# harvardinformatics/IMCoalHMM

Measured on AMD Instinct MI355X. Metric: alignment columns/sec (forward pass), 20-state isolation HMM, higher is better.
Workload: dtype f64

## Files before the change

### imcoalhmm_amd/csrc/imcoal_fwd.hip

```cpp
#include <hip/hip_runtime.h>

#include <algorithm>
#include <cerrno>
#include <climits>
#include <cmath>
#include <cstdint>
#include <cstdio>
#include <cstdlib>
#include <cstring>
#include <list>
#include <atomic>
#include <chrono>
#include <map>
#include <set>
#include <memory>
#include <mutex>
#include <condition_variable>
#include <string>
#include <vector>

#include <unistd.h>

#include "../../include/imcoal_fwd.h"
#include "kernels_plain.hpp"
// ... 59 lines not shown
    uint16_t *d_left = nullptr, *d_right = nullptr;
    uint16_t *d_order = nullptr;
    std::vector<uint16_t> order;
    std::vector<int> depth;
    uint64_t trained_on = 0;
    pid_t pid = 0;
    ~DictDev()
    {
        if (pid == getpid()) { dev_free(d_left); dev_free(d_right); dev_free(d_order); }
    }
};

struct Ev3 { hipEvent_t a, b, c; };

struct Ctx {
    pid_t pid = 0;
    int device = -1;
    bool ready = false;
    hipStream_t stream = nullptr;
    int cus = 256;
    uint64_t next_obs_id = 1, next_dict_id = 1;
    size_t seg_override = 0;
    int compression = 1;
    int kernel_pref = 0;
    bool profile = false;
    bool rank1_handoff = true;
    int blocked_variant = 4;
    int wide_blocked = -1;
    int z4_stream = -1;
    bool table_pairs = true;
    int table_triples = -1;
    bool table_split = true;
    int table_split_max = -1;
    bool xcd_affine = true;
    int fuse_tail = 1;
    bool fuse_head = true;
    bool pack_table = true;
    bool guard = false;
    bool use_graphs = false;
    std::vector<Ev3> events;
    std::map<int, std::shared_ptr<DictDev>> dicts;
    uint64_t last_plan[8] = {0, 0, 0, 0, 0, 0, 0, 0};
    uint64_t r1_checked = 0, r1_collapsed = 0;
    std::string last_kernels;
} g;

void drop_plans();
void reset_kernel_attributes();
void model_release();

int ensure_ctx()
{
    const pid_t me = getpid();
    if (g.ready && g.pid == me) return IMC_OK;
    if (g.ready && g.pid != me)
        return fail(IMC_ERR_HIP, "libimcoal_fwd was initialised in the parent process before fork(): fork the chain "
                                 "processes before the first imc_* call of the parent, or use the spawn start method");
    int n = 0;
    if (hipGetDeviceCount(&n) != hipSuccess || n <= 0)
        return fail(IMC_ERR_NODEVICE, "no HIP device available (libimcoal_fwd has no CPU fallback)");
    if (g.device < 0) {
        int cur = 0;
        if (hipGetDevice(&cur) != hipSuccess) cur = 0;
        g.device = cur;
    }
    if (g.device >= n) return fail(IMC_ERR_NODEVICE, "requested device index out of range");
    HIP_TRY(hipSetDevice(g.device));
    hipDeviceProp_t prop;
    HIP_TRY(hipGetDeviceProperties(&prop, g.device));
    if (std::strncmp(prop.gcnArchName, "gfx950", 6) != 0)
        return fail(IMC_ERR_NODEVICE, std::string("device is ") + prop.gcnArchName + ", this library is built for gfx950 only");
    g.cus = prop.multiProcessorCount > 0 ? prop.multiProcessorCount : 256;
    HIP_TRY(hipStreamCreateWithFlags(&g.stream, hipStreamNonBlocking));
    g.use_graphs = std::getenv("IMC_GRAPH") != nullptr;
    if (const char *gd = std::getenv("IMC_GUARD")) g.guard = std::atoi(gd) != 0;
    if (const char *bv = std::getenv("IMC_BLOCKED")) { const int v = std::atoi(bv); if (v >= 2 && v <= 5) g.blocked_variant = v; }
    if (const char *r1 = std::getenv("IMC_RANK1")) g.rank1_handoff = std::atoi(r1) != 0;
    if (const char *pt = std::getenv("IMC_PACK_TABLE")) g.pack_table = std::atoi(pt) != 0;
    if (const char *tp = std::getenv("IMC_TABLE_PAIRS")) g.table_pairs = std::atoi(tp) != 0;
    if (const char *fh = std::getenv("IMC_FUSE_HEAD")) g.fuse_head = std::atoi(fh) != 0;
    if (const char *ts = std::getenv("IMC_TABLE_SPLIT")) g.table_split = std::atoi(ts) != 0;
    if (const char *tm = std::getenv("IMC_TABLE_SPLIT_MAX")) g.table_split_max = std::max(0, std::atoi(tm));
    if (const char *tt = std::getenv("IMC_TABLE_TRIPLES")) g.table_triples = std::atoi(tt) != 0 ? 1 : 0;
    if (const char *ft = std::getenv("IMC_FUSE_TAIL")) g.fuse_tail = std::max(0, std::min(2, std::atoi(ft)));
    if (const char *xa = std::getenv("IMC_XCD_AFFINE")) g.xcd_affine = std::atoi(xa) != 0;
    if (const char *wb = std::getenv("IMC_WIDE_BLOCKED")) { const int v = std::atoi(wb); if (v >= -1 && v <= 1) g.wide_blocked = v; }
    if (const char *zs = std::getenv("IMC_Z4_STREAM")) { const int v = std::atoi(zs); if (v >= -1 && v <= 1) g.z4_stream = v; }
    g.pid = me;
    g.ready = true;
    return IMC_OK;
}

struct GuardRec { hipDeviceptr_t va; size_t va_size; hipMemGenericAllocationHandle_t handle; hipDeviceptr_t map; size_t map_size; };
std::map<void *, GuardRec> &g_guard = *new std::map<void *, GuardRec>();

hipError_t dev_alloc(void **p, size_t bytes)
{
    bytes = std::max<size_t>(bytes, 16);
    if (!g.guard) return hipMalloc(p, bytes);
    hipMemAllocationProp prop{};
    prop.type = hipMemAllocationTypePinned;
    prop.location.type = hipMemLocationTypeDevice;
    prop.location.id = g.device;
    size_t gran = 0;
    hipError_t e = hipMemGetAllocationGranularity(&gran, &prop, hipMemAllocationGranularityMinimum);
    if (e != hipSuccess || gran == 0) return e != hipSuccess ? e : hipErrorUnknown;
    GuardRec r{};
    r.map_size = (bytes + gran - 1) / gran * gran;
    r.va_size = r.map_size + 2 * gran;
    e = hipMemAddressReserve(&r.va, r.va_size, gran, nullptr, 0);
    if (e != hipSuccess) return e;
    e = hipMemCreate(&r.handle, r.map_size, &prop, 0);
    if (e != hipSuccess) { (void)hipMemAddressFree(r.va, r.va_size); return e; }
    r.map = (hipDeviceptr_t)((char *)r.va + gran);
    e = hipMemMap(r.map, r.map_size, 0, r.handle, 0);
    if (e == hipSuccess) {
        hipMemAccessDesc ad{};
        ad.location = prop.location;
// ... 10 lines not shown

void dev_free(void *p)
{
    if (!p) return;
    auto it = g_guard.find(p);
    if (it == g_guard.end()) { (void)hipFree(p); return; }
    (void)hipDeviceSynchronize();
    (void)hipMemUnmap(it->second.map, it->second.map_size);
    (void)hipMemRelease(it->second.handle);
    g_guard.erase(it);
}

}

struct imc_obs {
    uint64_t id;
    pid_t pid;
    int device;
    int nsym;
    size_t L;
    uint8_t *d_sym;
    bool wide_raw;
    std::shared_ptr<DictDev> dict;
    uint8_t *d_tok[imc::kNumLevels];
    bool wide[imc::kNumLevels];
    size_t ntok[imc::kNumLevels];
    int alphabet[imc::kNumLevels];
    std::vector<uint32_t> tok_count[imc::kNumLevels];
};

namespace {

constexpr size_t OBS_PAD = 256;

hipError_t upload_padded(const uint8_t *host, size_t n, uint8_t **dptr)
{
    const size_t bytes = ((n + OBS_PAD - 1) / OBS_PAD) * OBS_PAD + OBS_PAD;
    hipError_t e = dev_alloc((void **)dptr, bytes);
    if (e != hipSuccess) return e;
    e = hipMemsetAsync(*dptr, 0, bytes, g.stream);
    if (e == hipSuccess && n) e = hipMemcpyAsync(*dptr, host, n, hipMemcpyHostToDevice, g.stream);
    if (e == hipSuccess) e = hipStreamSynchronize(g.stream);
    return e;
}

void release_tokens(imc_obs *o)
{
    for (int l = 0; l < imc::kNumLevels; ++l) {
        bool alias = false;
        for (int m = 0; m < l; ++m) alias |= (o->d_tok[m] == o->d_tok[l]);
        if (o->d_tok[l] && !alias) dev_free(o->d_tok[l]);
    }
    for (int l = 0; l < imc::kNumLevels; ++l) {
        o->d_tok[l] = nullptr; o->wide[l] = false; o->ntok[l] = 0; o->alphabet[l] = o->nsym; o->tok_count[l].clear();
    }
    o->dict.reset();
}

void obs_release(imc_obs *o)
{
    dev_free(o->d_sym);
    release_tokens(o);
}

size_t wide_min_count(size_t sample_tokens)
{
// ... 141 lines not shown
    return IMC_OK;
}


using ChainFn = void (*)(const ChainDesc *, int, const uint32_t *, uint32_t, uint32_t, const double *, const int *,
                         const int *, uint32_t, double *, int *, double *, int);

struct KernelChoice {
    int R, G, NP, VPW, minw;
    void (*plain)(PropArgs);
    void (*zip)(PropArgs);
    size_t (*zip_lds)(int);
    ChainFn chain;
    bool zip_attr_set;
    void (*big_table_raw)(BigArgs);
    void (*big_table_level)(BigArgs, const uint16_t *, int);
    void (*big_prop)(BigArgs, const BigBlock *);
    int big_prop_waves;
    void (*big_vec)(BigArgs, const BigBlock *, int, int);
    void (*big_vec_tail)(BigArgs, const BigBlock *, int, int);
    int big_vec_waves;
    int big_nslab;
    size_t big_lds;
    void (*zip2)(BigArgs);
    size_t (*zip2_lds)(int);
    bool zip2_attr_set;
    bool plain_attr_set = false;
    void (*zip3)(BigArgs) = nullptr;
    size_t (*zip3_lds)(int) = nullptr;
    bool zip3_attr_set = false;
    void (*zip4)(BigArgs) = nullptr;
    void (*zip4w)(BigArgs) = nullptr;
    void (*zip4s)(BigArgs) = nullptr, (*zip4sw)(BigArgs) = nullptr;
    void (*zip4_raw)(BigArgs) = nullptr;
    void (*zip4_level)(BigArgs, int, int) = nullptr;
    void (*zip4_level2)(BigArgs, const int4 *, int, int, const double *) = nullptr;
    void (*zip4_level2_first)(BigArgs, const int4 *, int, int, const double *) = nullptr;
    void (*zip4_level2_split)(BigArgs, const int4 *, int, int, const double *) = nullptr;
    void (*zip4_level2_split_first)(BigArgs, const int4 *, int, int, const double *) = nullptr;
    void (*zip4_level3)(BigArgs, const int4 *, int, int, const double *) = nullptr;
    void (*zip4_level3_first)(BigArgs, const int4 *, int, int, const double *) = nullptr;
    size_t (*zip4_level3_lds)(size_t) = nullptr;
    size_t (*zip4_lds)(int, int) = nullptr;
    int (*zip4_max_hot)(int, size_t) = nullptr;
    int tok_doubles = 0;
    int z4_waves = Z2WAVES;
    bool wide_blocked = false;
    int z4_slots() const { return z4_waves * 4; }
    bool chain_self_emax = false;
    bool zip4_attr_set = false, zip4w_attr_set = false, zip4s_attr_set = false, zip4sw_attr_set = false, zip4_attr_l3 = false;
    bool use3() const;
    size_t blocked_lds(int A) const { return use3() ? zip3_lds(A) : zip2_lds(A); }
};

template <int R, int G, int MW>
KernelChoice make_kc()
{
    constexpr int NP = R * G;
    KernelChoice k{R, G, NP, 64 / G, MW, k_propagate<R, G, MW>, k_zpropagate<R, G>, &ZipGeom<R, G>::lds_bytes,
                   k_chain<NP, (NP <= 12 ? 6 : NP <= 24 ? 4 : NP <= 32 ? 3 : NP <= 64 ? 2 : 1)>, false, nullptr, nullptr, nullptr, 0, nullptr, nullptr, 0, 0, 0, nullptr, nullptr, false};
    k.chain_self_emax = true;
    if constexpr (NP % 4 == 0 && NP <= 24) {
        k.zip2 = k_zpropagate2<NP / 4>;
        k.zip2_lds = &Zip2Geom<NP / 4>::lds_bytes;
        k.zip3 = k_zpropagate3<NP / 4>;
        k.zip3_lds = &Zip3Geom<NP / 4>::lds_bytes;
        k.tok_doubles = Zip3Geom<NP / 4>::TOK;
        if constexpr (NP <= 24) {
            k.zip4 = k_zpropagate4<NP / 4, false, true>;
            k.zip4w = k_zpropagate4<NP / 4, true, true>;
            k.zip4s = k_zpropagate4<NP / 4, false, false>;
            k.zip4sw = k_zpropagate4<NP / 4, true, false>;
            k.zip4_raw = k_z4_raw<NP / 4>;
            k.zip4_level = k_z4_level<NP / 4>;
            k.zip4_level2 = k_z4_level2<NP / 4, false>;
            k.zip4_level2_first = k_z4_level2<NP / 4, true>;
            k.zip4_level2_split = k_z4_level2<NP / 4, false, Z4_SPLIT_WAVES>;
            k.zip4_level2_split_first = k_z4_level2<NP / 4, true, Z4_SPLIT_WAVES_FIRST>;
            k.zip4_level3 = k_z4_level3<NP / 4, false>;
            k.zip4_level3_first = k_z4_level3<NP / 4, true>;
            k.zip4_level3_lds = &Z4L3Geom<NP / 4>::lds_bytes;
            k.zip4_lds = &Zip4Geom<NP / 4>::lds_bytes;
            k.zip4_max_hot = &Zip4Geom<NP / 4>::max_hot;
        }
    }
    if constexpr (NP == 28 || NP == 32) {
        k.tok_doubles = Zip3Geom<NP / 4>::TOK;
        k.zip4s = k_zpropagate4<NP / 4, false, false>;
        k.zip4sw = k_zpropagate4<NP / 4, true, false>;
        k.zip4_raw = k_z4_raw<NP / 4>;
        k.zip4_level = k_z4_level<NP / 4>;
        k.zip4_lds = &Zip4Geom<NP / 4>::lds_bytes;
        k.z4_waves = Zip4Shape<NP / 4>::WAVES;
        k.wide_blocked = true;
    }
    return k;
}

template <int NT, int NSLAB>
KernelChoice make_big()
{
    constexpr int NP = 16 * NT;
    constexpr bool dealt = NT > 4 && NT % 4 != 0;
    void (*prop)(BigArgs, const BigBlock *) = k_big_propagate<NT, NSLAB>;
    if constexpr (dealt) prop = k_big_propagate_s<NT, NSLAB>;
    return KernelChoice{0, NT, NP, 0, 1, nullptr, nullptr, nullptr, k_chain<NP, 0>, false, k_big_table_raw<NT>,
                        k_big_table_level<NT>, prop, dealt ? BS_WAVES : NT, k_big_vector<NT, false>, k_big_vector<NT, true>, BigVec<NT>::WAVES, NSLAB,
                        BigSlab<NT, NSLAB>::bytes, nullptr, nullptr, false};
}

bool KernelChoice::use3() const { return zip3 && g.blocked_variant >= 3; }

KernelChoice kChoices[] = {
    make_kc<4, 1, 2>(), make_kc<4, 2, 2>(), make_kc<4, 3, 2>(), make_kc<4, 4, 2>(), make_kc<4, 5, 2>(),
    make_kc<3, 8, 2>(), make_kc<2, 14, 2>(), make_kc<2, 16, 2>(), make_kc<2, 20, 1>(), make_kc<1, 48, 1>(),
    make_kc<1, 56, 1>(), make_kc<1, 64, 1>(),
    make_big<6, 1>(), make_big<7, 1>(), make_big<8, 2>(), make_big<9, 3>(), make_big<10, 2>(), make_big<12, 3>(), make_big<14, 7>(),
    make_big<16, 8>(),
};
constexpr int IMC_MAX_N = 256;

KernelChoice kMidChoices[] = {make_big<2, 1>(), make_big<3, 1>(), make_big<4, 1>()};

KernelChoice *choose_kernel(int N, bool prefer_gemm)
{
    if (prefer_gemm && N > 24 && N <= 64)
        for (auto &k : kMidChoices)
            if (k.NP >= N) return &k;
    for (auto &k : kChoices)
        if (k.NP >= N) return &k;
    return nullptr;
}

void reset_kernel_attributes()
{
    for (auto &k : kChoices) k.zip4_attr_l3 = k.zip_attr_set = k.zip2_attr_set = k.zip3_attr_set = k.zip4_attr_set = k.zip4w_attr_set = k.zip4s_attr_set = k.zip4sw_attr_set = k.plain_attr_set = false;
    for (auto &k : kMidChoices) k.zip4_attr_l3 = k.zip_attr_set = k.zip2_attr_set = k.zip3_attr_set = k.zip4_attr_set = k.zip4w_attr_set = k.zip4s_attr_set = k.zip4sw_attr_set = k.plain_attr_set = false;
}


struct Group {
    bool big = false;
    bool bigvec = false;
    bool zip2 = false;
    std::vector<uint32_t> seg_ids, seg_out;
    std::vector<Z2Block> blocks;
    std::vector<BigBlock> big_blocks;
    BigBlock *d_big_blocks = nullptr;
    uint32_t *d_seg_ids = nullptr, *d_seg_out = nullptr;
    Z2Block *d_blocks = nullptr;
    bool zip4 = false;
    bool wide_tokens = false;
    bool stream_table = false;
    int n_hot = 0;
    std::vector<uint16_t> hot;
    uint16_t *d_hot = nullptr;
    uint16_t *d_tab_order = nullptr;
    int *d_tab_lvl = nullptr;
    int4 *d_tab_desc = nullptr;
    int4 *d_tab_desc2 = nullptr;
    std::vector<std::pair<int, int>> tab2;
    std::vector<Z2Tail> tails;
    Z2Tail *d_tails = nullptr;
    double *d_tailX = nullptr;
    int *d_tailE = nullptr, *d_tail_arrive = nullptr;
    int tail_stride = 0;
    int4 *d_tab_desc3 = nullptr;
    std::vector<std::pair<int, int>> tab3;
    std::vector<int> tab_lvl;
// ... 367 lines not shown
                size_t lmax = 0;
                for (size_t L : lens) lmax = std::max(lmax, L);
                const double np2 = (double)kc->NP * kc->NP, per_cu_steps = (double)total * B / (double)g.cus;
                const double cost_vec = std::max((double)lmax * (np2 / 4.5 + 1500.0), per_cu_steps * matvec_step_cycles(np2, gr.A));
                double cost_gemm = std::max(16.0, per_cu_steps) * gemm_cu_step_cycles(kc->NP);
                if (g.rank1_handoff && !g.seg_override && gr.seglen >= R1_MIN_SEGLEN) {
                    const HandoffEstimate he = estimate_handoff((double)gr.seglen, std::max(1.0, (double)total / gr.seglen), B,
                                                                (double)handoff_head(gr), kc->NP, kc->big_nslab, gr.A, g.cus);
                    if (he.m) cost_gemm = std::min(cost_gemm, he.cycles);
                }
                if (std::getenv("IMC_DEBUG"))
                    std::fprintf(stderr, "[imc] plan: GEMM chain seg %zu cost %.3g cycles; mat-vec chain cost %.3g cycles\n",
                                 gr.seglen, cost_gemm, cost_vec);
                if (!op_mode && (g.kernel_pref == 1 || (g.kernel_pref == 0 && (cost_vec < cost_gemm || lmax <= gr.seglen)))) {
                    gr.bigvec = true;
                    gr.seglen = std::max<size_t>(16, round_up(lmax, 16));
                }
                if (gr.zip) gr.model_us = gr.model_tab_us + (gr.bigvec ? cost_vec : cost_gemm) / 2200.0;
            } else {
                double cost_vec = 0.0;
                size_t seg_vec;
                if (gr.zip) {
                    const double lds_cycles = ((double)kc->R * kc->NP / 2 + kc->NP / 2.0) * 4.0 + kc->R * 6.0 + 40.0;
                    seg_vec = choose_seglen(lens, N, B, kc->VPW, (double)g.cus * ZWAVES, lds_cycles * ZWAVES, &cost_vec);
                } else {
                    seg_vec = choose_seglen(lens, N, B, kc->VPW, (double)g.cus * 4.0 * kc->minw,
                                            kc->minw * 1.7 * (4.0 * kc->R * kc->NP + 16.0), &cost_vec);
                }
                gr.seglen = seg_vec;
                if ((kc->zip2 || (wide && gr.zip4)) && g.kernel_pref != 1 && (gr.zip4 || kc->blocked_lds(gr.A) <= LDS_BUDGET) && (gr.zip || (S == gr.A && S <= imc::kByteAlphabet))) {
                    const int SL = kc->z4_slots(), WV = kc->z4_waves;
                    size_t total = 0;
                    for (size_t L : lens) total += L;
                    const bool two_per_cu = gr.zip4 && kc->use3() && kc->NP <= 12 &&
                                            z4_streamed((double)B * (gr.A + 1) * kc->tok_doubles * 8.0, B);
                    const double rows = (double)g.cus * SL * (two_per_cu ? 2.0 : 1.0);
                    const double rb = kc->NP / 4.0;
                    const double step_cycles = (mfma() ? 25.5 * rb * rb * rb * 0.55 : 5.8 * rb * rb * kc->NP) * (two_per_cu ? 1.85 : 1.0);
                    size_t seg_blk = 16;
                    double slots = 0.0, cost_blk = 1e300;
                    const bool can_pack = mfma() && !op_mode;
                    auto rows_used = [&](size_t sg) {
                        double r = 0.0, singles = 0.0;
                        for (size_t L : lens) {
                            if (!L) continue;
                            const double nseg = std::ceil((double)L / (double)sg);
                            if (nseg <= 1.0 && can_pack) singles += 1.0;
                            else r += std::ceil(nseg / SL) * SL;
                        }
                        return r + std::ceil(singles / SL) * SL;
                    };
                    size_t lmax = 0;
                    for (size_t L : lens) lmax = std::max(lmax, L);
                    std::vector<size_t> cands;
                    for (int rounds = 1; rounds <= 16; ++rounds) {
                        const double target = std::max((double)SL, std::floor(rows * rounds / B));
                        size_t sg = std::max<size_t>(16, round_up((size_t)std::ceil((double)total / target), Z2GRAN));
                        int it = 0;
                        for (; it < 1024 && rows_used(sg) > target && sg < lmax + 16; ++it) sg += Z2GRAN;
                        if (rows_used(sg) > target) continue;
                        cands.push_back(sg);
                    }
                    for (size_t u = 1; u <= 8; ++u)
                        cands.push_back(std::max<size_t>(16, round_up((lmax + SL * u - 1) / (SL * u), Z2GRAN)));
                    {
                        std::vector<size_t> sorted(lens);
                        std::sort(sorted.begin(), sorted.end());
                        const size_t med = sorted[sorted.size() / 2];
                        for (size_t u = 1; u <= 4; ++u)
                            cands.push_back(std::max<size_t>(16, round_up((med + SL * u - 1) / (SL * u), Z2GRAN)));
                        for (size_t fixed_len : {16, 32, 48, 64, 96, 128, 192}) cands.push_back(fixed_len);
                        if (can_pack)
                            for (size_t qi : {sorted.size() / 2, sorted.size() * 9 / 10, sorted.size() - 1})
                                cands.push_back(std::max<size_t>(16, round_up(sorted[qi], Z2GRAN)));
                    }
                    for (size_t sg : cands) {
                        const double table = !mfma() ? (double)(gr.A - S) * (400.0 + (double)kc->NP * kc->NP * kc->NP / 64.0)
                                             : gr.zip4 ? 9000.0 : 2600.0 * std::min(12.0, (double)(gr.A - S));
                        const double fixed = table + 5.0 * (WV / 4.0) * step_cycles;
                        for (size_t cand : {sg, round_up(sg, 16)}) {
                            const double u = rows_used(cand);
                            double c = std::ceil(u * B / rows) * ((double)cand * (WV / 4.0) * step_cycles + fixed + (cand % 16 ? 7700.0 : 0.0));
                            if (can_pack && cand >= lmax) c *= 1.15;
                            if (c < cost_blk) { cost_blk = c; seg_blk = cand; slots = u; }
                        }
                    }
                    if (std::getenv("IMC_DEBUG"))
                        std::fprintf(stderr, "[imc] plan: vector kernel seg %zu cost %.3g cycles; blocked kernel seg %zu slots %.0f cost %.3g cycles\n",
                                     seg_vec, cost_vec, seg_blk, slots, cost_blk);
                    const bool vec_fits = !gr.zip || kc->zip_lds(gr.A) <= LDS_BUDGET;
                    if (g.kernel_pref == 2 || cost_blk < cost_vec || !vec_fits || gr.zip4) { gr.zip2 = true; gr.seglen = seg_blk; }
                }
                if (gr.zip && !gr.zip2) gr.model_us = gr.model_tab_us + cost_vec / 2200.0;
            }
            if (g.seg_override) gr.seglen = round_up(std::max<size_t>(g.seg_override, 16), 16);
            if (gr.bigvec)
                for (size_t L : lens) gr.bigvec = gr.bigvec && L <= gr.seglen && !op_mode;
            if (gr.big && !gr.bigvec && g.rank1_handoff && gr.seglen >= R1_MIN_SEGLEN) {
                double cols = 0.0, toks = 0.0;
                for (int f : gr.chunks) { cols += (double)chunks[f]->L; toks += (double)(gr.zip ? chunks[f]->ntok[gr.level] : chunks[f]->L); }
                const double span = toks > 0.0 ? cols / toks : 1.0;
                const size_t head = handoff_head(gr);
                const double nseg = std::max(1.0, toks / (double)gr.seglen);
                if (g.seg_override) {
                    if (gr.seglen >= 4 * R1_MIN_HEAD) {
                        gr.rank1 = true;
                        gr.head_len = (int)round_up(gr.seglen / 4, 16);
                        gr.checkpoints.assign(1, gr.head_len);
                    }
                } else {
                    const int best_m = estimate_handoff((double)gr.seglen, nseg, B, (double)head, kc->NP, kc->big_nslab, gr.A, g.cus).m;
                    if (best_m) {
                        gr.rank1 = true;
                        gr.head_len = (int)head;
                        gr.seglen = std::max<size_t>(16, round_up(gr.seglen / best_m, 16));
                        size_t c = round_up(std::max<size_t>(64, (size_t)(R1_HEAD_MIN_COLUMNS / span)), 16);
                        while ((int)gr.checkpoints.size() < R1_MAX_ROUNDS && c + gr.seglen / 8 < gr.seglen) {
                            gr.checkpoints.push_back((int)c);
                            const size_t step = (double)c * span < R1_DENSE_COLUMNS ? c / 8 : c / 2;
                            c = round_up(c + std::max<size_t>(16, step), 16);
                        }
                        if (gr.checkpoints.empty()) gr.rank1 = false;
                    }
                }
            }
        }
    }

    void cut_segments()
    {
        chunk_seg.assign(n_chunks + 1, 0);
        for (int f = 0; f < n_chunks; ++f) {
            chunk_seg[f] = (uint32_t)segs.size();
            const Group &gr = p->groups[chunk_group[f]];
            const size_t L = gr.zip ? chunks[f]->ntok[gr.level] : chunks[f]->L;
            const uint8_t *base = gr.zip ? chunks[f]->d_tok[gr.level] : chunks[f]->d_sym;
            if (!L) continue;
            const size_t K0 = (L + gr.seglen - 1) / gr.seglen;
            const size_t sl = round_up((L + K0 - 1) / K0, gr.zip2 ? Z2GRAN : 16);
            for (size_t off = 0, k = 0; off < L; off += sl, ++k) {
                const bool wide = gr.zip ? chunks[f]->wide[gr.level] : chunks[f]->wide_raw;
                const bool fst = k == 0 && !op_mode;
                segs.push_back(SegDesc{base + off * (wide ? 2 : 1), (uint32_t)std::min(sl, L - off),
                                       (fst ? SEG_FIRST : 0u) | (wide ? SEG_WIDE : 0u)});
                seg_first.push_back(fst);
            }
        }
        chunk_seg[n_chunks] = (uint32_t)segs.size();
    }

    int make_units()
    {
        chunk_units.assign(n_chunks, {});
        for (int f = 0; f < n_chunks; ++f) {
            const Group &gr = p->groups[chunk_group[f]];
            const uint32_t step = gr.zip2 ? (uint32_t)kc->z4_slots() : 1u;
            for (uint32_t sid = chunk_seg[f]; sid < chunk_seg[f + 1]; sid += step)
                chunk_units[f].push_back({sid, std::min(step, chunk_seg[f + 1] - sid)});
        }
        chunk_unit.assign(n_chunks + 1, 0);
        for (int f = 0; f < n_chunks; ++f) chunk_unit[f + 1] = chunk_unit[f] + (uint32_t)chunk_units[f].size();
        unit_vec0.assign(chunk_unit[n_chunks], 0);
        unit_first.assign(chunk_unit[n_chunks], 0);
        for (Group &gr : p->groups) {
            gr.vec_begin = (uint32_t)vecs.size();
            for (int f : gr.chunks) {
                gr.stream_len += gr.zip ? chunks[f]->ntok[gr.level] : chunks[f]->L;
                for (size_t u = 0; u < chunk_units[f].size(); ++u) {
                    const uint32_t sid = chunk_units[f][u].first, ns = chunk_units[f][u].second;
                    const uint32_t uid = chunk_unit[f] + (uint32_t)u;
                    const bool fst = seg_first[sid] != 0;
                    unit_first[uid] = fst;
// ... 593 lines not shown
                        head = false;
                        HIP_TRY(hipGetLastError());
                    }
                } else if (g.table_pairs && gr.d_tab_desc2 && kc->zip4_level2) {
                    bool head = fuse_head;
                    const size_t split_max = g.table_split_max >= 0 ? (size_t)g.table_split_max : (size_t)4 * g.cus;
                    for (const auto &lc : gr.tab2) {
                        if (g.table_split && (size_t)lc.second * B <= split_max) {
                            if (head)
                                hipLaunchKernelGGL(kc->zip4_level2_split_first, dim3((unsigned)(lc.second + Z4_SPLIT_WAVES_FIRST - 1) / Z4_SPLIT_WAVES_FIRST, (unsigned)B),
                                                   dim3(Z4_SPLIT_WAVES_FIRST * 64), p->pstride * 8, stream, ba,
                                                   (const int4 *)gr.d_tab_desc2, lc.first, lc.second, (const double *)p->h_params_dev[p->slot]);
                            else
                                hipLaunchKernelGGL(kc->zip4_level2_split, dim3((unsigned)(lc.second + Z4_SPLIT_WAVES - 1) / Z4_SPLIT_WAVES, (unsigned)B),
                                                   dim3(Z4_SPLIT_WAVES * 64), 0, stream, ba,
                                                   (const int4 *)gr.d_tab_desc2, lc.first, lc.second, (const double *)nullptr);
                            split_used = true;
                        } else if (head)
                            hipLaunchKernelGGL(kc->zip4_level2_first, dim3((unsigned)(lc.second + 3) / 4, (unsigned)B), dim3(64),
                                               p->pstride * 8, stream, ba,
                                               (const int4 *)gr.d_tab_desc2, lc.first, lc.second, (const double *)p->h_params_dev[p->slot]);
                        else
                            hipLaunchKernelGGL(kc->zip4_level2, dim3((unsigned)(lc.second + 3) / 4, (unsigned)B), dim3(64), 0, stream, ba,
                                               (const int4 *)gr.d_tab_desc2, lc.first, lc.second, (const double *)nullptr);
                        head = false;
                        HIP_TRY(hipGetLastError());
                    }
                } else
                for (int d = 0; d < gr.tab_nlvl; ++d) {
                    const int first = gr.tab_lvl[d], count = gr.tab_lvl[d + 1] - first;
                    hipLaunchKernelGGL(kc->zip4_level, dim3((unsigned)(count + 3) / 4, (unsigned)B), dim3(64), 0, stream, ba, first, count);
                    HIP_TRY(hipGetLastError());
                }
                void (*scan)(BigArgs) = gr.stream_table ? (gr.wide_tokens ? kc->zip4sw : kc->zip4s) : (gr.wide_tokens ? kc->zip4w : kc->zip4);
                bool &attr4 = gr.stream_table ? (gr.wide_tokens ? kc->zip4sw_attr_set : kc->zip4s_attr_set)
                                              : (gr.wide_tokens ? kc->zip4w_attr_set : kc->zip4_attr_set);
                if (!attr4) {
                    HIP_TRY(hipFuncSetAttribute((const void *)scan, hipFuncAttributeMaxDynamicSharedMemorySize, (int)LDS_BUDGET));
                    attr4 = true;
                }
                IMC_MARK_A();
                dim3 scan_grid(ba.n_group_segs, (unsigned)B);
                if (g.xcd_affine && B > 1) {
                    int first = 0, wg = 0;
                    auto phase = [&](int sets, int n_sets_total) {
                        ba.ph_begin[ba.n_phases] = wg; ba.ph_first[ba.n_phases] = first; ba.ph_sets[ba.n_phases] = sets;
                        ++ba.n_phases;
                        const int nb = (int)ba.n_group_segs;
                        wg += sets >= 8 ? 8 * nb * (n_sets_total / 8) : 8 * ((nb + 8 / sets - 1) / (8 / sets));
                        first += n_sets_total;
                    };
                    if (B >= 8) phase(8, B / 8 * 8);
                    for (int sets : {4, 2, 1})
                        if ((B % 8) & sets) phase(sets, sets);
                    scan_grid = dim3((unsigned)wg);
                }
                hipLaunchKernelGGL(scan, scan_grid, dim3(kc->z4_waves * 64), kc->zip4_lds(gr.A, gr.n_hot), stream, ba);
                note(std::string("k_zpropagate4<") + std::to_string(NP / 4) + (gr.wide_tokens ? ",16" : "") + (gr.stream_table ? ",streamed>" : ">") + strm);
                lp[4] = gr.seglen; lp[5] += gr.vsteps * (uint64_t)B; lp[6] += gr.stream_len; lp[7] = std::max(lp[7], (uint64_t)gr.A);
                HIP_TRY(hipGetLastError());
                continue;
            }
            const bool v3 = kc->use3();
            bool &attr_set = v3 ? kc->zip3_attr_set : kc->zip2_attr_set;
            if (!attr_set) {
                HIP_TRY(hipFuncSetAttribute((const void *)(v3 ? kc->zip3 : kc->zip2), hipFuncAttributeMaxDynamicSharedMemorySize,
                                            (int)LDS_BUDGET));
                attr_set = true;
            }
            size_t lds3 = kc->blocked_lds(gr.A);
            if (direct_params) { ba.params_src = p->h_params_dev[p->slot]; lds3 = ((lds3 + 15) & ~(size_t)15) + p->pstride * 8; }
            hipLaunchKernelGGL(v3 ? kc->zip3 : kc->zip2, dim3(ba.n_group_segs, (unsigned)B), dim3(Z2WAVES * 64), lds3, stream, ba);
            note(std::string(v3 ? "k_zpropagate3<" : "k_zpropagate2<") + std::to_string(NP / 4) + ">" + strm);
            if (gr.zip) { lp[4] = gr.seglen; lp[5] += gr.vsteps * (uint64_t)B; lp[6] += gr.stream_len; lp[7] = std::max(lp[7], (uint64_t)gr.A); }
            else { lp[2] = gr.seglen; lp[3] += gr.vsteps * (uint64_t)B; }
        } else if (gr.zip) {
            const size_t lds = kc->zip_lds(gr.A);
            if (!kc->zip_attr_set) {
                HIP_TRY(hipFuncSetAttribute((const void *)kc->zip, hipFuncAttributeMaxDynamicSharedMemorySize,
                                            (int)LDS_BUDGET));
                kc->zip_attr_set = true;
            }
            const uint32_t vpb = (uint32_t)(ZWAVES * kc->VPW);
            dim3 grid((gr.n_vecs + vpb - 1) / vpb, (unsigned)B);
            hipLaunchKernelGGL(kc->zip, grid, dim3(ZWAVES * 64), lds, stream, a);
            note("k_zpropagate<" + std::to_string(kc->R) + "," + std::to_string(kc->G) + ">" + strm);
            lp[4] = gr.seglen; lp[5] += gr.vsteps * (uint64_t)B; lp[6] += gr.stream_len; lp[7] = std::max(lp[7], (uint64_t)gr.A);
        } else {
            const uint32_t vpb = (uint32_t)(WPB * kc->VPW);
            dim3 grid((gr.n_vecs + vpb - 1) / vpb, (unsigned)B);
            const size_t lds = ((size_t)WPB * kc->VPW * NP + (size_t)S * NP) * 8;
// ... 1036 lines not shown
```

### imcoalhmm_amd/csrc/kernels_zip4.hpp

```cpp
#pragma once
#include "kernels_zip3.hpp"

template <int NT>
struct Zip4Shape {
    static constexpr int WAVES = NT <= 6 ? Z2WAVES : 4;
    static constexpr int SLOTS = WAVES * 4;
    static constexpr bool SLOT_MAP = NT <= 6;
};

template <int NT>
struct Zip4Geom {
    using G3 = Zip3Geom<NT>;
    static constexpr int TOK = G3::TOK;
    static constexpr int SLOTS = Zip4Shape<NT>::SLOTS;
    static constexpr int MAPS = Zip4Shape<NT>::SLOT_MAP ? 2 : 1;
    static constexpr int slots(int H) { return (H + 1 > SLOTS + 1 ? H + 1 : SLOTS + 1); }
    static constexpr size_t lds_bytes(int A, int H) { return (size_t)slots(H) * TOK * 8 + (size_t)(MAPS * (A + 2) + 64) * 4 + 16; }
    static constexpr int max_hot(int A, size_t budget)
    {
        const size_t fixed = (size_t)(MAPS * (A + 2) + 64) * 4 + 16;
        const size_t n = budget > fixed ? (budget - fixed) / ((size_t)TOK * 8) : 0;
        return n > 1 ? (int)n - 1 : 0;
    }
};

template <int NT>
__device__ __forceinline__ void zip4_step_regs(const double (&Pin)[NT][NT], double (&Pout)[NT][NT], const double (&Areg)[NT][NT])
{
#pragma unroll
    for (int I = 0; I < NT; ++I)
#pragma unroll
        for (int K = 0; K < NT; ++K)
#pragma unroll
            for (int J = 0; J < NT; ++J)
                Pout[I][J] = __builtin_amdgcn_mfma_f64_4x4x4f64(Areg[I][K], Pin[K][J], K == 0 ? 0.0 : Pout[I][J], 0, 0, 0);
}

template <int NT>
__device__ __forceinline__ void zip4_load_row_global(double (&a)[NT], const double *Gz, int I, int lo, int lx)
{
// ... 458 lines not shown
    const double *Cz = C + (size_t)max(cur.s, 0) * TOK, *Cn = C + (size_t)max(nxt.s, 0) * TOK;
#pragma unroll
    for (int I = 0; I < NT; ++I) {
        double an[NT], av[NT];
        if constexpr (HYB) {
            if (I + 1 < NT) zip3_load_row<NT>(an, Cz, I + 1, lo, lx);
            else zip3_load_row<NT>(an, Cn, 0, lo, lx);
        }
#pragma unroll
        for (int K = 0; K < NT; ++K) av[K] = cur_cold ? pre[I % ROWS][K] : al[K];
        __builtin_amdgcn_sched_barrier(0);
#pragma unroll
        for (int K = 0; K < NT; ++K)
#pragma unroll
            for (int J = 0; J < NT; ++J)
                Pout[I][J] = __builtin_amdgcn_mfma_f64_4x4x4f64(av[K], Pin[K][J], K == 0 ? 0.0 : Pout[I][J], 0, 0, 0);
        __builtin_amdgcn_sched_barrier(0);
        if (I + ROWS < NT) zip4_load_row_global<NT>(pre[I % ROWS], Gt + (size_t)cur.tok * TOK, I + ROWS, lo, lx);
        else zip4_load_row_global<NT>(pre[I % ROWS], Gn, I + ROWS - NT, lo, lx);
        if constexpr (HYB) {
#pragma unroll
            for (int K = 0; K < NT; ++K) al[K] = an[K];
        }
    }
}

#ifdef IMC_Z4_TIMING
__device__ long long g_z4_dbg[1024 * 8 * 3];
#define Z4_STAMP(k_) do { if (threadIdx.x == 0 && blockIdx.x < 1024 && blockIdx.y == 0) g_z4_dbg[blockIdx.x * 8 + (k_)] = wall_clock64(); } while (0)
#else
#define Z4_STAMP(k_) do { } while (0)
#endif

template <int NT, bool WIDE, bool HYB>
__global__ __launch_bounds__(Zip4Shape<NT>::WAVES * 64, Zip4Shape<NT>::WAVES / 4) void k_zpropagate4(BigArgs a)
{
    constexpr int TB = WIDE ? 2 : 1;
    using Geo = Zip3Geom<NT>;
    using G4 = Zip4Geom<NT>;
    constexpr int SLOTS = Zip4Shape<NT>::SLOTS;
    constexpr bool SLOT_MAP = Zip4Shape<NT>::SLOT_MAP;
    static_assert(SLOT_MAP || !HYB, "the hybrid form needs the slot map");
    constexpr int NP = Geo::NP, TOK = Geo::TOK, THREADS = Zip4Shape<NT>::WAVES * 64;
    extern __shared__ __attribute__((aligned(16))) double lds[];
    const int H = HYB ? a.n_hot : 0;
    double *C = lds;
    int *cex = reinterpret_cast<int *>(C + (size_t)G4::slots(H) * TOK);
    int *slot_of = cex + a.A + 2;
    int *xex = SLOT_MAP ? slot_of + a.A + 2 : slot_of;

    const int tid = threadIdx.x;
    int b = (int)blockIdx.y, bx = (int)blockIdx.x;
    if (a.n_phases > 0) {
        int ph = 0;
        while (ph + 1 < a.n_phases && (int)blockIdx.x >= a.ph_begin[ph + 1]) ++ph;
        const int local = (int)blockIdx.x - a.ph_begin[ph], xcd = local & 7, turn = local >> 3, nb = (int)a.n_group_segs;
        const int sets = a.ph_sets[ph];
        if (sets >= 8) {
            b = a.ph_first[ph] + xcd + 8 * (turn / nb);
            bx = turn % nb;
        } else {
            b = a.ph_first[ph] + xcd % sets;
            bx = turn * (8 / sets) + xcd / sets;
            if (bx >= nb) return;
        }
    }
    const double *pp = a.params + (size_t)b * a.pstride;
    const double *pi_p = pp;
    const double *Etg = pp + a.PP + (size_t)a.PP * a.PP;
    const double *Gt = a.Ctab + (size_t)b * (a.A + 1) * TOK;
    const int *Gc = a.cex + (size_t)b * (a.A + 1);
    const int IDENT = a.A;
    const double *Gi = Gt + (size_t)IDENT * TOK;

    Z4_STAMP(0);
    for (int z = tid; z <= a.A; z += THREADS) { cex[z] = Gc[z]; if constexpr (SLOT_MAP) slot_of[z] = -1; }
    if constexpr (HYB) {
        __syncthreads();
        for (int k = tid; k <= H; k += THREADS) slot_of[k < H ? (int)a.hot[k] : IDENT] = k;
        for (int idx = tid; idx < (H + 1) * (TOK / 2); idx += THREADS) {
            const int k = idx / (TOK / 2), w = idx - k * (TOK / 2);
            const int z = k < H ? (int)a.hot[k] : IDENT;
            reinterpret_cast<double2 *>(C + (size_t)k * TOK)[w] = reinterpret_cast<const double2 *>(Gt + (size_t)z * TOK)[w];
        }
    }
    __syncthreads();

    Z4_STAMP(1);
    const int lane = tid & 63;
    const int q = lane >> 4, bq = (lane >> 2) & 3, r = lane & 3;
    const int lo = (q * 4 + r) * Geo::NTE, lx = q * 4 + r;
    const Z2Block blk = a.blocks[bx];
    const int slot = (tid >> 6) * 4 + bq;
    const bool valid = slot < (int)blk.n;
    const uint32_t seg = blk.seg0 + (valid ? slot : ((slot & ~3) < (int)blk.n ? (slot & ~3) : 0));
    const SegDesc sd = a.segs[seg];
    const int len = valid ? (int)sd.len : 0;
    const bool first = (sd.first & SEG_FIRST) != 0;
    const uint8_t *tokp = sd.obs;
    typedef const __attribute__((address_space(1))) uint8_t *gptr;
    typedef uint32_t u32x4 __attribute__((ext_vector_type(4)));
    typedef const __attribute__((address_space(1))) u32x4 *gptr4;
    typedef const __attribute__((address_space(1))) uint32_t *gptr1;
    const gptr tokg = (gptr)tokp;

    double P[NT][NT], Q[NT][NT];
    {
        const int tok0 = (valid && first) ? seg_token(tokp, WIDE, 0) : 0;
#pragma unroll
        for (int K = 0; K < NT; ++K)
#pragma unroll
            for (int J = 0; J < NT; ++J) {
                const int i = 4 * K + q, c = 4 * J + r;
                double v;
                if (first) v = (c == 0 && i < a.N) ? pi_p[i] * Etg[(size_t)tok0 * a.PP + i] : 0.0;
                else v = (i == c && i < a.N) ? 1.0 : 0.0;
                P[K][J] = valid ? v : 0.0;
            }
    }
    int ex = 0;
    const int maxlen = wave_max_i32(len);
// ... 36 lines not shown
        }
        ex += t0.ce + t1.ce;
    };
    constexpr int PER = WIDE ? 8 : 16;
    auto masked_run = [&](int bi, int u0, int n) __attribute__((always_inline)) {
        uint4 ob = make_uint4(0u, 0u, 0u, 0u);
        if (bi * RESCALE_EVERY + u0 < len) {
            const u32x4 v = *(gptr4)(tokg + ((size_t)bi * RESCALE_EVERY + u0) * TB);
            ob = make_uint4(v.x, v.y, v.z, v.w);
        }
        const int live = len - bi * RESCALE_EVERY - u0;
        const int dead0 = (first && bi == 0 && u0 == 0) ? 0 : -1;
        const unsigned long long lo64 = (unsigned long long)ob.y << 32 | ob.x, hi64 = (unsigned long long)ob.w << 32 | ob.z;
        auto tok_of = [&](int v) __attribute__((always_inline)) {
            const unsigned long long h = v < PER / 2 ? lo64 : hi64;
            const int tk = WIDE ? (int)((h >> (16 * (v & 3))) & 0xffffull) : (int)((h >> (8 * (v & 7))) & 0xffull);
            return (v < live && v != dead0 && v < PER) ? tk : IDENT;
        };
        Z4Tok c0 = mk(tok_of(0)), c1 = mk(tok_of(1));
        prime(c0, c1);
#pragma unroll 1
        for (int v = 0; v < n; v += 2) {
            const Z4Tok c2 = mk(tok_of(v + 2)), c3 = mk(tok_of(v + 3));
            two_steps(c0, c1, c2, c3);
            c0 = c2;
            c1 = c3;
        }
    };
    auto masked_block = [&](int bi, int npos) __attribute__((always_inline)) {
#pragma unroll 1
        for (int u0 = 0; u0 < npos; u0 += PER) masked_run(bi, u0, min(PER, npos - u0));
        zip3_rescale<NT>(P, ex);
    };
    if (nfull == 0 && maxlen > 0) masked_block(0, min(RESCALE_EVERY, (maxlen + 1) & ~1));
    Z4_STAMP(2);
    if (nfull > 0) {
        constexpr int NW = 4 * TB;
        constexpr uint32_t TM = WIDE ? 0xffffu : 0xffu;
        auto load_words = [&](int bi, uint32_t (&w)[NW]) __attribute__((always_inline)) {
            gptr4 src = (gptr4)(tokg + (size_t)bi * RESCALE_EVERY * TB);
            const u32x4 x = src[0];
            w[0] = x.x; w[1] = x.y; w[2] = x.z; w[3] = x.w;
            if constexpr (WIDE) {
                const u32x4 y = src[1];
                w[4] = y.x; w[5] = y.y; w[6] = y.z; w[7] = y.w;
            }
        };
        uint32_t cw[NW];
        load_words(0, cw);
        Z4Tok c0 = mk(first ? IDENT : (int)(cw[0] & TM));
        prime(c0, mk(WIDE ? (int)(cw[0] >> 16) : (int)((cw[0] >> 8) & TM)));
        for (int bi = 0; bi < nfull; ++bi) {
            const bool more = bi + 1 < nfull;
            const int bn = more ? bi + 1 : bi;
            const uint32_t nfirst = *(gptr1)(tokg + (size_t)bn * RESCALE_EVERY * TB);
#pragma unroll
            for (int g4 = 0; g4 < 4; ++g4) {
                int t1, t2, t3, t4;
                if constexpr (WIDE) {
                    const uint32_t wa = cw[0], wb = cw[1];
#pragma unroll
                    for (int k = 0; k + 2 < NW; ++k) cw[k] = cw[k + 2];
                    t1 = (int)(wa >> 16); t2 = (int)(wb & TM); t3 = (int)(wb >> 16);
                } else {
                    const uint32_t wa = cw[0];
#pragma unroll
                    for (int k = 0; k + 1 < NW; ++k) cw[k] = cw[k + 1];
                    t1 = (int)((wa >> 8) & TM); t2 = (int)((wa >> 16) & TM); t3 = (int)(wa >> 24);
                }
                t4 = g4 < 3 ? (int)(cw[0] & TM) : more ? (int)(nfirst & TM) : IDENT;
                const uint32_t w5 = g4 < 3 ? cw[0] : nfirst;
                const int t5 = (g4 < 3 || more) ? (WIDE ? (int)(w5 >> 16) : (int)((w5 >> 8) & TM)) : IDENT;
                if (g4 == 3) load_words(bn, cw);
                const Z4Tok c1 = mk(t1), c2 = mk(t2), c3 = mk(t3);
                two_steps(c0, c1, c2, c3);
                const Z4Tok c4 = mk(t4), c5 = mk(t5);
                two_steps(c2, c3, c4, c5);
                c0 = c4;
            }
            zip3_rescale<NT>(P, ex);
        }
    }
    Z4_STAMP(3);
    for (int bi = max(1, nfull); bi * RESCALE_EVERY < maxlen; ++bi)
        masked_block(bi, min(RESCALE_EVERY, (maxlen - bi * RESCALE_EVERY + 1) & ~1));
    zip3_rescale<NT>(P, ex);
    Z4_STAMP(4);
#ifdef IMC_Z4_TIMING
    if ((threadIdx.x & 63) == 0 && blockIdx.x < 1024 && blockIdx.y == 0) g_z4_dbg[1024 * 8 + blockIdx.x * 8 + (threadIdx.x >> 6)] = wall_clock64();
#endif

    if (blk.first == 2) {
        if (valid && r == 0) {
            const size_t gvp = (size_t)b * a.n_vecs_total + blk.out_vec0 + slot;
#pragma unroll
            for (int K = 0; K < NT; ++K)
                if (4 * K + q < a.N) a.P[gvp * NP + 4 * K + q] = P[K][0];
            if (q == 0) a.EX[gvp] = ex;
        }
        return;
    }

    zip3_fold<NT, HYB, true, SLOTS>(P, ex, C, xex, (int)blk.n, slot, tid >> 6, lo, lx);

    Z4_STAMP(5);
#ifdef IMC_Z4_TIMING
    if (threadIdx.x == 0 && blockIdx.x < 1024 && blockIdx.y == 0) g_z4_dbg[blockIdx.x * 8 + 7] = (long long)nfull * 1000000 + maxlen;
#endif
    if (slot == 0) {
        const size_t gv = (size_t)b * a.n_vecs_total + blk.out_vec0;
        double *Pout = a.P + gv * NP;
        if (blk.first) {
            if (r == 0) {
#pragma unroll
                for (int K = 0; K < NT; ++K)
                    if (4 * K + q < a.N) Pout[4 * K + q] = P[K][0];
            }
            if (q == 0 && r == 0) a.EX[gv] = ex;
        } else {
#pragma unroll
            for (int K = 0; K < NT; ++K)
#pragma unroll
                for (int J = 0; J < NT; ++J) {
                    const int i = 4 * K + q, c = 4 * J + r;
                    if (i < a.N && c < a.N) Pout[(size_t)i * NP + c] = P[K][J];
                }
            if (q == 0) {
#pragma unroll
                for (int J = 0; J < NT; ++J)
                    if (4 * J + r < a.N) a.EX[gv + 4 * J + r] = ex;
            }
        }
    }
    if (a.tail) zip3_tail<NT, SLOTS>(a, P, ex, C, xex, b, bx, slot, lo, lx);
}
```

Baseline: 397.7 billion.

## Pipeline zip4 scan token loads with LDS fill and handle partial tail inline

Restructures the zip4 scan kernel so the first token words are loaded and the chain primed before the LDS table fill, overlapping global latency with the setup. A partial final block is now processed inside the main loop from registers instead of the generic masked path. The segment planner can use 2-token granularity for wide tokens and drops the masked-tail penalty from its cost model. The old path stays reachable through IMC_SCAN_TAIL=0. The trade-off is more code complexity and register pressure, and a different segmentation plan.

```diff
diff --git a/imcoalhmm_amd/csrc/imcoal_fwd.hip b/imcoalhmm_amd/csrc/imcoal_fwd.hip
--- a/imcoalhmm_amd/csrc/imcoal_fwd.hip
+++ b/imcoalhmm_amd/csrc/imcoal_fwd.hip
@@ -115,6 +115,7 @@
     int table_triples = -1;
     bool table_split = true;
     int table_split_max = -1;
+    int scan_tail = 2;
     bool xcd_affine = true;
     int fuse_tail = 1;
     bool fuse_head = true;
@@ -167,6 +168,7 @@
     if (const char *tt = std::getenv("IMC_TABLE_TRIPLES")) g.table_triples = std::atoi(tt) != 0 ? 1 : 0;
     if (const char *ft = std::getenv("IMC_FUSE_TAIL")) g.fuse_tail = std::max(0, std::min(2, std::atoi(ft)));
     if (const char *xa = std::getenv("IMC_XCD_AFFINE")) g.xcd_affine = std::atoi(xa) != 0;
+    if (const char *st = std::getenv("IMC_SCAN_TAIL")) g.scan_tail = std::max(0, std::min(2, std::atoi(st)));
     if (const char *wb = std::getenv("IMC_WIDE_BLOCKED")) { const int v = std::atoi(wb); if (v >= -1 && v <= 1) g.wide_blocked = v; }
     if (const char *zs = std::getenv("IMC_Z4_STREAM")) { const int v = std::atoi(zs); if (v >= -1 && v <= 1) g.z4_stream = v; }
     g.pid = me;
@@ -243,6 +245,8 @@
 namespace {
 
 constexpr size_t OBS_PAD = 256;
+
+size_t z2gran(bool wide16) { return wide16 && g.scan_tail >= 2 ? 2 : Z2GRAN; }
 
 hipError_t upload_padded(const uint8_t *host, size_t n, uint8_t **dptr)
 {
@@ -450,6 +454,8 @@
     void (*zip4)(BigArgs) = nullptr;
     void (*zip4w)(BigArgs) = nullptr;
     void (*zip4s)(BigArgs) = nullptr, (*zip4sw)(BigArgs) = nullptr;
+    void (*zip4_mt[4])(BigArgs) = {nullptr, nullptr, nullptr, nullptr};
+    bool zip4_mt_attr_set[4] = {false, false, false, false};
     void (*zip4_raw)(BigArgs) = nullptr;
     void (*zip4_level)(BigArgs, int, int) = nullptr;
     void (*zip4_level2)(BigArgs, const int4 *, int, int, const double *) = nullptr;
@@ -489,6 +495,10 @@
             k.zip4w = k_zpropagate4<NP / 4, true, true>;
             k.zip4s = k_zpropagate4<NP / 4, false, false>;
             k.zip4sw = k_zpropagate4<NP / 4, true, false>;
+            k.zip4_mt[0] = k_zprop4_masked_tail<NP / 4, false, true>;
+            k.zip4_mt[1] = k_zprop4_masked_tail<NP / 4, true, true>;
+            k.zip4_mt[2] = k_zprop4_masked_tail<NP / 4, false, false>;
+            k.zip4_mt[3] = k_zprop4_masked_tail<NP / 4, true, false>;
             k.zip4_raw = k_z4_raw<NP / 4>;
             k.zip4_level = k_z4_level<NP / 4>;
             k.zip4_level2 = k_z4_level2<NP / 4, false>;
@@ -506,6 +516,8 @@
         k.tok_doubles = Zip3Geom<NP / 4>::TOK;
         k.zip4s = k_zpropagate4<NP / 4, false, false>;
         k.zip4sw = k_zpropagate4<NP / 4, true, false>;
+        k.zip4_mt[2] = k_zprop4_masked_tail<NP / 4, false, false>;
+        k.zip4_mt[3] = k_zprop4_masked_tail<NP / 4, true, false>;
         k.zip4_raw = k_z4_raw<NP / 4>;
         k.zip4_level = k_z4_level<NP / 4>;
         k.zip4_lds = &Zip4Geom<NP / 4>::lds_bytes;
@@ -552,7 +564,9 @@
 
 void reset_kernel_attributes()
 {
+    for (auto &k : kChoices) for (bool &f : k.zip4_mt_attr_set) f = false;
     for (auto &k : kChoices) k.zip4_attr_l3 = k.zip_attr_set = k.zip2_attr_set = k.zip3_attr_set = k.zip4_attr_set = k.zip4w_attr_set = k.zip4s_attr_set = k.zip4sw_attr_set = k.plain_attr_set = false;
+    for (auto &k : kMidChoices) for (bool &f : k.zip4_mt_attr_set) f = false;
     for (auto &k : kMidChoices) k.zip4_attr_l3 = k.zip_attr_set = k.zip2_attr_set = k.zip3_attr_set = k.zip4_attr_set = k.zip4w_attr_set = k.zip4s_attr_set = k.zip4sw_attr_set = k.plain_attr_set = false;
 }
 
@@ -986,6 +1000,7 @@
                     const int SL = kc->z4_slots(), WV = kc->z4_waves;
                     size_t total = 0;
                     for (size_t L : lens) total += L;
+                    const size_t gran = z2gran(gr.wide_tokens);
                     const bool two_per_cu = gr.zip4 && kc->use3() && kc->NP <= 12 &&
                                             z4_streamed((double)B * (gr.A + 1) * kc->tok_doubles * 8.0, B);
                     const double rows = (double)g.cus * SL * (two_per_cu ? 2.0 : 1.0);
@@ -1009,32 +1024,33 @@
                     std::vector<size_t> cands;
                     for (int rounds = 1; rounds <= 16; ++rounds) {
                         const double target = std::max((double)SL, std::floor(rows * rounds / B));
-                        size_t sg = std::max<size_t>(16, round_up((size_t)std::ceil((double)total / target), Z2GRAN));
+                        size_t sg = std::max<size_t>(16, round_up((size_t)std::ceil((double)total / target), gran));
                         int it = 0;
-                        for (; it < 1024 && rows_used(sg) > target && sg < lmax + 16; ++it) sg += Z2GRAN;
+                        for (; it < 1024 && rows_used(sg) > target && sg < lmax + 16; ++it) sg += gran;
                         if (rows_used(sg) > target) continue;
                         cands.push_back(sg);
                     }
                     for (size_t u = 1; u <= 8; ++u)
-                        cands.push_back(std::max<size_t>(16, round_up((lmax + SL * u - 1) / (SL * u), Z2GRAN)));
+                        cands.push_back(std::max<size_t>(16, round_up((lmax + SL * u - 1) / (SL * u), gran)));
                     {
                         std::vector<size_t> sorted(lens);
                         std::sort(sorted.begin(), sorted.end());
                         const size_t med = sorted[sorted.size() / 2];
                         for (size_t u = 1; u <= 4; ++u)
-                            cands.push_back(std::max<size_t>(16, round_up((med + SL * u - 1) / (SL * u), Z2GRAN)));
+                            cands.push_back(std::max<size_t>(16, round_up((med + SL * u - 1) / (SL * u), gran)));
                         for (size_t fixed_len : {16, 32, 48, 64, 96, 128, 192}) cands.push_back(fixed_len);
                         if (can_pack)
                             for (size_t qi : {sorted.size() / 2, sorted.size() * 9 / 10, sorted.size() - 1})
-                                cands.push_back(std::max<size_t>(16, round_up(sorted[qi], Z2GRAN)));
+                                cands.push_back(std::max<size_t>(16, round_up(sorted[qi], gran)));
                     }
                     for (size_t sg : cands) {
                         const double table = !mfma() ? (double)(gr.A - S) * (400.0 + (double)kc->NP * kc->NP * kc->NP / 64.0)
                                              : gr.zip4 ? 9000.0 : 2600.0 * std::min(12.0, (double)(gr.A - S));
                         const double fixed = table + 5.0 * (WV / 4.0) * step_cycles;
+                        const double masked = gr.zip4 && kc->NP != 24 && g.scan_tail >= 2 ? 0.0 : 7700.0;
                         for (size_t cand : {sg, round_up(sg, 16)}) {
                             const double u = rows_used(cand);
-                            double c = std::ceil(u * B / rows) * ((double)cand * (WV / 4.0) * step_cycles + fixed + (cand % 16 ? 7700.0 : 0.0));
+                            double c = std::ceil(u * B / rows) * ((double)cand * (WV / 4.0) * step_cycles + fixed + (cand % 16 ? masked : 0.0));
                             if (can_pack && cand >= lmax) c *= 1.15;
                             if (c < cost_blk) { cost_blk = c; seg_blk = cand; slots = u; }
                         }
@@ -1091,7 +1107,7 @@
             const uint8_t *base = gr.zip ? chunks[f]->d_tok[gr.level] : chunks[f]->d_sym;
             if (!L) continue;
             const size_t K0 = (L + gr.seglen - 1) / gr.seglen;
-            const size_t sl = round_up((L + K0 - 1) / K0, gr.zip2 ? Z2GRAN : 16);
+            const size_t sl = round_up((L + K0 - 1) / K0, gr.zip2 ? z2gran(gr.wide_tokens) : 16);
             for (size_t off = 0, k = 0; off < L; off += sl, ++k) {
                 const bool wide = gr.zip ? chunks[f]->wide[gr.level] : chunks[f]->wide_raw;
                 const bool fst = k == 0 && !op_mode;
@@ -1751,9 +1767,12 @@
                     hipLaunchKernelGGL(kc->zip4_level, dim3((unsigned)(count + 3) / 4, (unsigned)B), dim3(64), 0, stream, ba, first, count);
                     HIP_TRY(hipGetLastError());
                 }
-                void (*scan)(BigArgs) = gr.stream_table ? (gr.wide_tokens ? kc->zip4sw : kc->zip4s) : (gr.wide_tokens ? kc->zip4w : kc->zip4);
-                bool &attr4 = gr.stream_table ? (gr.wide_tokens ? kc->zip4sw_attr_set : kc->zip4s_attr_set)
-                                              : (gr.wide_tokens ? kc->zip4w_attr_set : kc->zip4_attr_set);
+                const int mt = (gr.stream_table ? 2 : 0) + (gr.wide_tokens ? 1 : 0);
+                void (*scan)(BigArgs) = g.scan_tail == 0 ? kc->zip4_mt[mt]
+                                        : gr.stream_table ? (gr.wide_tokens ? kc->zip4sw : kc->zip4s) : (gr.wide_tokens ? kc->zip4w : kc->zip4);
+                bool &attr4 = g.scan_tail == 0 ? kc->zip4_mt_attr_set[mt]
+                              : gr.stream_table ? (gr.wide_tokens ? kc->zip4sw_attr_set : kc->zip4s_attr_set)
+                                                : (gr.wide_tokens ? kc->zip4w_attr_set : kc->zip4_attr_set);
                 if (!attr4) {
                     HIP_TRY(hipFuncSetAttribute((const void *)scan, hipFuncAttributeMaxDynamicSharedMemorySize, (int)LDS_BUDGET));
                     attr4 = true;
@@ -1775,7 +1794,7 @@
                     scan_grid = dim3((unsigned)wg);
                 }
                 hipLaunchKernelGGL(scan, scan_grid, dim3(kc->z4_waves * 64), kc->zip4_lds(gr.A, gr.n_hot), stream, ba);
-                note(std::string("k_zpropagate4<") + std::to_string(NP / 4) + (gr.wide_tokens ? ",16" : "") + (gr.stream_table ? ",streamed>" : ">") + strm);
+                note(std::string("k_zpropagate4<") + std::to_string(NP / 4) + (gr.wide_tokens ? ",16" : "") + (gr.stream_table ? ",streamed" : "") + (g.scan_tail == 0 ? ",masked-tail>" : ">") + strm);
                 lp[4] = gr.seglen; lp[5] += gr.vsteps * (uint64_t)B; lp[6] += gr.stream_len; lp[7] = std::max(lp[7], (uint64_t)gr.A);
                 HIP_TRY(hipGetLastError());
                 continue;
diff --git a/imcoalhmm_amd/csrc/kernels_zip4.hpp b/imcoalhmm_amd/csrc/kernels_zip4.hpp
--- a/imcoalhmm_amd/csrc/kernels_zip4.hpp
+++ b/imcoalhmm_amd/csrc/kernels_zip4.hpp
@@ -6,6 +6,7 @@
     static constexpr int WAVES = NT <= 6 ? Z2WAVES : 4;
     static constexpr int SLOTS = WAVES * 4;
     static constexpr bool SLOT_MAP = NT <= 6;
+    static constexpr bool PIPE = NT != 6;
 };
 
 template <int NT>
@@ -530,8 +531,10 @@
 #define Z4_STAMP(k_) do { } while (0)
 #endif
 
-template <int NT, bool WIDE, bool HYB>
-__global__ __launch_bounds__(Zip4Shape<NT>::WAVES * 64, Zip4Shape<NT>::WAVES / 4) void k_zpropagate4(BigArgs a)
+__device__ __forceinline__ uint32_t zip4_pick(bool c, uint32_t x, uint32_t y) { return c ? x : y; }
+
+template <int NT, bool WIDE, bool HYB, bool PIPE>
+__device__ __forceinline__ void zip4_scan(const BigArgs &a)
 {
     constexpr int TB = WIDE ? 2 : 1;
     using Geo = Zip3Geom<NT>;
@@ -572,19 +575,22 @@
     const double *Gi = Gt + (size_t)IDENT * TOK;
 
     Z4_STAMP(0);
-    for (int z = tid; z <= a.A; z += THREADS) { cex[z] = Gc[z]; if constexpr (SLOT_MAP) slot_of[z] = -1; }
-    if constexpr (HYB) {
+    auto fill_lds = [&]() __attribute__((always_inline)) {
+        for (int z = tid; z <= a.A; z += THREADS) { cex[z] = Gc[z]; if constexpr (SLOT_MAP) slot_of[z] = -1; }
+        if constexpr (HYB) {
+            __syncthreads();
+            for (int k = tid; k <= H; k += THREADS) slot_of[k < H ? (int)a.hot[k] : IDENT] = k;
+            for (int idx = tid; idx < (H + 1) * (TOK / 2); idx += THREADS) {
+                const int k = idx / (TOK / 2), w = idx - k * (TOK / 2);
+                const int z = k < H ? (int)a.hot[k] : IDENT;
+                reinterpret_cast<double2 *>(C + (size_t)k * TOK)[w] = reinterpret_cast<const double2 *>(Gt + (size_t)z * TOK)[w];
+            }
+        }
         __syncthreads();
-        for (int k = tid; k <= H; k += THREADS) slot_of[k < H ? (int)a.hot[k] : IDENT] = k;
-        for (int idx = tid; idx < (H + 1) * (TOK / 2); idx += THREADS) {
-            const int k = idx / (TOK / 2), w = idx - k * (TOK / 2);
-            const int z = k < H ? (int)a.hot[k] : IDENT;
-            reinterpret_cast<double2 *>(C + (size_t)k * TOK)[w] = reinterpret_cast<const double2 *>(Gt + (size_t)z * TOK)[w];
-        }
-    }
-    __syncthreads();
-
-    Z4_STAMP(1);
+        Z4_STAMP(1);
+    };
+    if constexpr (!PIPE) fill_lds();
+
     const int lane = tid & 63;
     const int q = lane >> 4, bq = (lane >> 2) & 3, r = lane & 3;
     const int lo = (q * 4 + r) * Geo::NTE, lx = q * 4 + r;
@@ -687,27 +693,39 @@
         for (int u0 = 0; u0 < npos; u0 += PER) masked_run(bi, u0, min(PER, npos - u0));
         zip3_rescale<NT>(P, ex);
     };
+    constexpr int NW = 4 * TB;
+    constexpr int TPW = 4 / TB;
+    constexpr uint32_t TM = WIDE ? 0xffffu : 0xffu;
+    auto load_words = [&](int bi, uint32_t (&w)[NW], bool hi) __attribute__((always_inline)) {
+        gptr4 src = (gptr4)(tokg + (size_t)bi * RESCALE_EVERY * TB);
+        const u32x4 x = src[0];
+        w[0] = x.x; w[1] = x.y; w[2] = x.z; w[3] = x.w;
+        if constexpr (WIDE) {
+            const u32x4 y = src[hi ? 1 : 0];
+            w[4] = y.x; w[5] = y.y; w[6] = y.z; w[7] = y.w;
+        }
+    };
+    auto second_of = [&](uint32_t w) __attribute__((always_inline)) { return WIDE ? (int)(w >> 16) : (int)((w >> 8) & TM); };
+    uint32_t cw[NW];
+    if constexpr (PIPE) {
+        if (nfull > 0) {
+            load_words(0, cw, true);
+            if constexpr (!HYB) prime(Z4Tok{-1, 0, first ? IDENT : (int)(cw[0] & TM)}, Z4Tok{-1, 0, second_of(cw[0])});
+        }
+        fill_lds();
+    }
     if (nfull == 0 && maxlen > 0) masked_block(0, min(RESCALE_EVERY, (maxlen + 1) & ~1));
     Z4_STAMP(2);
+    int piped = 0;
     if (nfull > 0) {
-        constexpr int NW = 4 * TB;
-        constexpr uint32_t TM = WIDE ? 0xffffu : 0xffu;
-        auto load_words = [&](int bi, uint32_t (&w)[NW]) __attribute__((always_inline)) {
-            gptr4 src = (gptr4)(tokg + (size_t)bi * RESCALE_EVERY * TB);
-            const u32x4 x = src[0];
-            w[0] = x.x; w[1] = x.y; w[2] = x.z; w[3] = x.w;
-            if constexpr (WIDE) {
-                const u32x4 y = src[1];
-                w[4] = y.x; w[5] = y.y; w[6] = y.z; w[7] = y.w;
-            }
-        };
-        uint32_t cw[NW];
-        load_words(0, cw);
+        if constexpr (!PIPE) load_words(0, cw, true);
         Z4Tok c0 = mk(first ? IDENT : (int)(cw[0] & TM));
-        prime(c0, mk(WIDE ? (int)(cw[0] >> 16) : (int)((cw[0] >> 8) & TM)));
+        if constexpr (!PIPE || HYB) prime(c0, mk(second_of(cw[0])));
         for (int bi = 0; bi < nfull; ++bi) {
             const bool more = bi + 1 < nfull;
-            const int bn = more ? bi + 1 : bi;
+            const int left = len - (bi + 1) * RESCALE_EVERY;
+            const bool tail0 = more || (PIPE && left > 0), tail1 = more || (PIPE && left > 1);
+            const int bn = tail0 ? bi + 1 : bi;
             const uint32_t nfirst = *(gptr1)(tokg + (size_t)bn * RESCALE_EVERY * TB);
 #pragma unroll
             for (int g4 = 0; g4 < 4; ++g4) {
@@ -723,10 +741,10 @@
                     for (int k = 0; k + 1 < NW; ++k) cw[k] = cw[k + 1];
                     t1 = (int)((wa >> 8) & TM); t2 = (int)((wa >> 16) & TM); t3 = (int)(wa >> 24);
                 }
-                t4 = g4 < 3 ? (int)(cw[0] & TM) : more ? (int)(nfirst & TM) : IDENT;
+                t4 = g4 < 3 ? (int)(cw[0] & TM) : tail0 ? (int)(nfirst & TM) : IDENT;
                 const uint32_t w5 = g4 < 3 ? cw[0] : nfirst;
-                const int t5 = (g4 < 3 || more) ? (WIDE ? (int)(w5 >> 16) : (int)((w5 >> 8) & TM)) : IDENT;
-                if (g4 == 3) load_words(bn, cw);
+                const int t5 = (g4 < 3 || tail1) ? second_of(w5) : IDENT;
+                if (g4 == 3) load_words(bn, cw, !PIPE || more || left > RESCALE_EVERY / 2 || left <= 0);
                 const Z4Tok c1 = mk(t1), c2 = mk(t2), c3 = mk(t3);
                 two_steps(c0, c1, c2, c3);
                 const Z4Tok c4 = mk(t4), c5 = mk(t5);
@@ -735,9 +753,39 @@
             }
             zip3_rescale<NT>(P, ex);
         }
-    }
-    Z4_STAMP(3);
-    for (int bi = max(1, nfull); bi * RESCALE_EVERY < maxlen; ++bi)
+        if constexpr (PIPE) {
+            Z4_STAMP(3);
+            if (maxlen > nfull * RESCALE_EVERY) {
+                const int live = min(len - nfull * RESCALE_EVERY, RESCALE_EVERY);
+                const int npos = min(RESCALE_EVERY, (maxlen - nfull * RESCALE_EVERY + 1) & ~1);
+                auto tok_of = [&](int u) __attribute__((always_inline)) {
+                    const int wi = u / TPW;
+                    uint32_t w = zip4_pick(wi == 1, cw[1], cw[0]);
+                    w = zip4_pick(wi == 2, cw[2], w);
+                    w = zip4_pick(wi == 3, cw[3], w);
+                    if constexpr (WIDE) {
+                        w = zip4_pick(wi == 4, cw[NW - 4], w);
+                        w = zip4_pick(wi == 5, cw[NW - 3], w);
+                        w = zip4_pick(wi == 6, cw[NW - 2], w);
+                        w = zip4_pick(wi == 7, cw[NW - 1], w);
+                    }
+                    return u < live ? (int)((w >> ((u % TPW) * (8 * TB))) & TM) : IDENT;
+                };
+                Z4Tok c1 = mk(tok_of(1));
+#pragma unroll 1
+                for (int u = 0; u < npos; u += 2) {
+                    const Z4Tok c2 = mk(tok_of(u + 2)), c3 = mk(tok_of(u + 3));
+                    two_steps(c0, c1, c2, c3);
+                    c0 = c2;
+                    c1 = c3;
+                }
+                zip3_rescale<NT>(P, ex);
+                piped = 1;
+            }
+        }
+    }
+    if (!PIPE || nfull == 0) Z4_STAMP(3);
+    for (int bi = max(1, nfull + piped); bi * RESCALE_EVERY < maxlen; ++bi)
         masked_block(bi, min(RESCALE_EVERY, (maxlen - bi * RESCALE_EVERY + 1) & ~1));
     zip3_rescale<NT>(P, ex);
     Z4_STAMP(4);
@@ -789,3 +837,15 @@
     }
     if (a.tail) zip3_tail<NT, SLOTS>(a, P, ex, C, xex, b, bx, slot, lo, lx);
 }
+
+template <int NT, bool WIDE, bool HYB>
+__global__ __launch_bounds__(Zip4Shape<NT>::WAVES * 64, Zip4Shape<NT>::WAVES / 4) void k_zpropagate4(BigArgs a)
+{
+    zip4_scan<NT, WIDE, HYB, Zip4Shape<NT>::PIPE>(a);
+}
+
+template <int NT, bool WIDE, bool HYB>
+__global__ __launch_bounds__(Zip4Shape<NT>::WAVES * 64, Zip4Shape<NT>::WAVES / 4) void k_zprop4_masked_tail(BigArgs a)
+{
+    zip4_scan<NT, WIDE, HYB, false>(a);
+}
```

Result: no change. 398.7 billion, median of 2 (+0.3%).
